# Nikhil-Kulkarni/RayTrace-miniapp

Hardware: AMD Instinct MI355X
Metric: ray_steps_per_sec (higher is better)
Workload: dtype f32+f64

## Files before the change

include/rt_hip.h:

```cpp
#ifndef RT_HIP_H
#define RT_HIP_H

#include <stddef.h>
#include <stdint.h>

#ifdef __cplusplus
extern "C" {
#endif

#define RT_N_SUB 3
#define RT_N_FAILED_MAX 32

enum {
    RT_OK            = 0,
    RT_ERR_ARG       = 1,
    RT_ERR_NO_DEVICE = 2,
    RT_ERR_HIP       = 3,
    RT_ERR_NOMEM     = 4
};

typedef struct rt_ray {
    float x, y, a, b;
} rt_ray;

// ... 70 lines not shown
                             int ngy, const double *ga, int nga, const double *gb, int ngb,
                             int64_t first, int64_t stride, int64_t count);

int rt_hip_plan_run(rt_hip_plan *plan, void *stream, double *image_dev, double *iang_dev);

int rt_hip_plan_fetch(rt_hip_plan *plan, double *image, double *I_ang,
                      unsigned int *failure_code, rt_ray *failed_rays, int max_failed,
                      int *n_failed, rt_stats *stats);

int rt_hip_plan_kernel_ms(rt_hip_plan *plan, float *ms);

int rt_hip_plan_kernel_times(rt_hip_plan *plan, float *march_ms, float *freq_ms);

int rt_hip_plan_last_fused(rt_hip_plan *plan);

int rt_hip_plan_set_timing_ring(rt_hip_plan *plan, int n_runs);
int rt_hip_plan_ring_times(rt_hip_plan *plan, float *march_ms, float *freq_ms, int max_runs, int *n_runs);

double *rt_hip_plan_image_ptr(rt_hip_plan *plan);
double *rt_hip_plan_iang_ptr(rt_hip_plan *plan);

int rt_hip_plan_enable_probe(rt_hip_plan *plan, int on);
int rt_hip_plan_fetch_probe(rt_hip_plan *plan, float *gvl, float *evl, int32_t *ivl,
                            rt_ray *ray2, uint32_t *flags, uint32_t *steps);

int rt_hip_plan_set_exact_emission(rt_hip_plan *plan, int on);

int rt_hip_plan_set_step_factor(rt_hip_plan *plan, double c);

int rt_hip_plan_enable_path(rt_hip_plan *plan, int on);
// ... 18 lines not shown
```

raytrace-miniapp_amd/backend.py:

```python
from __future__ import annotations

import ctypes as C
import subprocess
import time
from pathlib import Path

import numpy as np

from . import cabi
from .problem import Problem

CSRC = Path(__file__).resolve().parent / "csrc"
LIB_PATH = CSRC / "librt_hip.so"


class RayTraceError(RuntimeError):
    """Raised where the reference calls RAY_ERROR (utilities/RayUtilityMacros.h:88-91)."""


def build_library(force: bool = False) -> Path:
    if force and LIB_PATH.exists():
        LIB_PATH.unlink()
    subprocess.run(["make", "-s", "-C", str(CSRC)], check=True)
    return LIB_PATH
# ... 157 lines not shown
        return torch.as_tensor(v, device=torch.device("cuda", self.device))

    def kernel_ms(self) -> float:
        ms = C.c_float(0)
        self.hl.check(self.hl.lib.rt_hip_plan_kernel_ms(self._h, C.byref(ms)), "rt_hip_plan_kernel_ms")
        return float(ms.value)

    def kernel_times(self) -> tuple:
        a, f = C.c_float(0), C.c_float(0)
        self.hl.check(self.hl.lib.rt_hip_plan_kernel_times(self._h, C.byref(a), C.byref(f)),
                      "rt_hip_plan_kernel_times")
        return float(a.value), float(f.value)

    def last_fused(self) -> bool:
        return bool(self.hl.lib.rt_hip_plan_last_fused(self._h))

    def set_timing_ring(self, n_runs: int) -> "Plan":
        self.hl.check(self.hl.lib.rt_hip_plan_set_timing_ring(self._h, int(n_runs)), "rt_hip_plan_set_timing_ring")
        self._ring = int(n_runs)
        return self

    def ring_times(self) -> list:
        n = getattr(self, "_ring", 0)
        if n < 1:
            return []
        a = np.zeros(n, np.float32)
        f = np.zeros(n, np.float32)
        got = C.c_int(0)
        self.hl.check(self.hl.lib.rt_hip_plan_ring_times(self._h, cabi._fp(a), cabi._fp(f), n, C.byref(got)),
                      "rt_hip_plan_ring_times")
# ... 163 lines not shown
```

raytrace-miniapp_amd/cabi.py:

```python
from __future__ import annotations

import ctypes as C

import numpy as np

RT_N_SUB = 3
RT_N_FAILED_MAX = 32

RT_OK, RT_ERR_ARG, RT_ERR_NO_DEVICE, RT_ERR_HIP, RT_ERR_NOMEM = range(5)

c_double_p = C.POINTER(C.c_double)
c_float_p = C.POINTER(C.c_float)


class RtRay(C.Structure):
    _fields_ = [("x", C.c_float), ("y", C.c_float), ("a", C.c_float), ("b", C.c_float)]


RAY_DTYPE = np.dtype([("x", "<f4"), ("y", "<f4"), ("a", "<f4"), ("b", "<f4")])


class RtBeam(C.Structure):
    _fields_ = [
        ("nx", C.c_int32), ("ny", C.c_int32), ("na", C.c_int32), ("nb", C.c_int32),
# ... 129 lines not shown
    lib.rt_hip_plan_set_ray_grid.argtypes = [vp, c_double_p, C.c_int, c_double_p, C.c_int,
                                             c_double_p, C.c_int, c_double_p, C.c_int,
                                             C.c_int64, C.c_int64, C.c_int64]
    lib.rt_hip_plan_set_ray_grid.restype = C.c_int
    lib.rt_hip_plan_run.argtypes = [vp, vp, vp, vp]
    lib.rt_hip_plan_run.restype = C.c_int
    lib.rt_hip_plan_fetch.argtypes = [vp, c_double_p, c_double_p, P(C.c_uint), P(RtRay), C.c_int,
                                      P(C.c_int), P(RtStats)]
    lib.rt_hip_plan_fetch.restype = C.c_int
    lib.rt_hip_plan_kernel_ms.argtypes = [vp, P(C.c_float)]
    lib.rt_hip_plan_kernel_ms.restype = C.c_int
    lib.rt_hip_plan_kernel_times.argtypes = [vp, P(C.c_float), P(C.c_float)]
    lib.rt_hip_plan_kernel_times.restype = C.c_int
    lib.rt_hip_plan_last_fused.argtypes = [vp]
    lib.rt_hip_plan_last_fused.restype = C.c_int
    lib.rt_hip_plan_set_timing_ring.argtypes = [vp, C.c_int]
    lib.rt_hip_plan_set_timing_ring.restype = C.c_int
    lib.rt_hip_plan_ring_times.argtypes = [vp, c_float_p, c_float_p, C.c_int, P(C.c_int)]
    lib.rt_hip_plan_ring_times.restype = C.c_int
    lib.rt_hip_plan_image_ptr.argtypes = [vp]
    lib.rt_hip_plan_image_ptr.restype = vp
    lib.rt_hip_plan_iang_ptr.argtypes = [vp]
    lib.rt_hip_plan_iang_ptr.restype = vp
    lib.rt_hip_plan_enable_probe.argtypes = [vp, C.c_int]
    lib.rt_hip_plan_enable_probe.restype = C.c_int
    lib.rt_hip_plan_fetch_probe.argtypes = [vp, c_float_p, c_float_p, P(C.c_int32), P(RtRay),
                                            P(C.c_uint32), P(C.c_uint32)]
    lib.rt_hip_plan_fetch_probe.restype = C.c_int
    lib.rt_hip_plan_set_exact_emission.argtypes = [vp, C.c_int]
    lib.rt_hip_plan_set_exact_emission.restype = C.c_int
# ... 10 lines not shown
    lib.rt_hip_plan_spectra_ptr.argtypes = [vp]
    lib.rt_hip_plan_spectra_ptr.restype = vp
    lib.rt_hip_calc_rays.argtypes = [C.c_int, C.c_int, C.c_double, P(RtGain), P(RtSeed), C.c_int, C.c_int, c_double_p,
                                     C.c_size_t, c_double_p, c_double_p, P(C.c_int32), P(RtStats)]
    lib.rt_hip_calc_rays.restype = C.c_int
    lib.rt_hip_plan_set_debug.argtypes = [vp, C.c_uint]
    lib.rt_hip_plan_set_debug.restype = C.c_int
    lib.rt_hip_plan_destroy.argtypes = [vp]
    lib.rt_hip_plan_destroy.restype = None


HIP_API_SYMBOLS = [
    "rt_hip_device_count", "rt_hip_last_error", "rt_hip_selftest", "rt_hip_image_loop", "rt_hip_multi_image_loop",
    "rt_hip_multi_last_mode", "rt_hip_ray_list_grid_dims", "rt_hip_host_libm_mode", "rt_hip_pool_trim", "rt_hip_plan_create",
    "rt_hip_plan_set_rays", "rt_hip_plan_set_ray_grid", "rt_hip_plan_run", "rt_hip_plan_fetch",
    "rt_hip_plan_kernel_ms", "rt_hip_plan_kernel_times", "rt_hip_plan_last_fused", "rt_hip_plan_set_timing_ring", "rt_hip_plan_ring_times", "rt_hip_plan_image_ptr", "rt_hip_plan_iang_ptr", "rt_hip_plan_enable_probe",
    "rt_hip_plan_fetch_probe", "rt_hip_plan_set_exact_emission", "rt_hip_plan_set_step_factor", "rt_hip_plan_enable_path",
    "rt_hip_plan_fetch_path", "rt_hip_plan_enable_spectra", "rt_hip_plan_fetch_spectra", "rt_hip_plan_spectra_ptr",
    "rt_hip_calc_rays", "rt_hip_plan_set_debug", "rt_hip_plan_destroy",
]
```

raytrace-miniapp_amd/csrc/rt_fused.hip:

```cpp
#pragma once
#include "rt_freq.hip"

namespace rt {

struct FusedLay {
    unsigned off_exp, off_iang, off_ctl, off_rem, off_nodes, off_buf;
    unsigned node_cap;
    unsigned n_free, per_wave;
    unsigned split, k_part;
    unsigned n_consumers, consumers_first;
};
struct FusedKArg {
    DevParams P;
    FreqKArg F;
    unsigned *tile_next;
    FusedLay lay;
};

constexpr int fused_wave_doubles(int maxq) { return 4 * XP_ROW + maxq * WAVE; }
template <bool BOUNDED, int SF, int MAXQ, bool EMIS = true>
__global__ void __launch_bounds__(1024) rt_fused_kernel(const FusedKArg A)
{
    extern __shared__ __align__(16) unsigned char lds_raw[];
#ifdef RT_WAVETIMES
    if (threadIdx.x == 0)
        atomicMin(&g_wt[2], __builtin_amdgcn_s_memrealtime());
#endif
    const FreqHot &H   = A.F.hot;
    const int n_ang    = H.n_ang;
    double *exp2_tab   = reinterpret_cast<double *>(lds_raw + A.lay.off_exp);
    double *lds_iang   = reinterpret_cast<double *>(lds_raw + A.lay.off_iang);
    unsigned *ctl      = reinterpret_cast<unsigned *>(lds_raw + A.lay.off_ctl);
    double *buf_free   = reinterpret_cast<double *>(lds_raw + A.lay.off_buf);
    const unsigned n_waves  = blockDim.x >> 6;
    const unsigned n_march  = n_waves - A.lay.n_consumers;
// ... 6 lines not shown
        lds_iang[c] = 0.0;
    for (unsigned c = threadIdx.x; c < n_waves * 32u; c += blockDim.x)
        reinterpret_cast<unsigned *>(lds_raw + A.lay.off_rem)[c] = 0u;
    if (threadIdx.x == 0) {
        ctl[0] = TILE_NONE;
        ctl[1] = n_march;
        ctl[2] = 0u;
        ctl[3] = 0u;
    }
    const TileList list{ &ctl[0], A.tile_next, reinterpret_cast<unsigned *>(lds_raw + A.lay.off_nodes), &ctl[3], A.lay.node_cap,
                         reinterpret_cast<unsigned *>(lds_raw + A.lay.off_rem) + wave_id * 32u,
                         &ctl[1], n_march, A.lay.split, A.lay.k_part };

    march_load_tables<true>(A.P, lds_raw);
    if (!consumer)
        march_wave<true, BOUNDED, true, EMIS ? 1 : 0>(A.P, lds_raw, list);

    const int lane = lane_id();
#ifdef RT_WAVETIMES
    const unsigned long long fu_left = __builtin_amdgcn_s_memrealtime();
    unsigned long long fu_first = 0, fu_tiles = 0;
#endif
    unsigned slot  = 0;
    if (lane == 0) {
        if (!consumer)
            __hip_atomic_fetch_add(&ctl[1], 0xffffffffu, __ATOMIC_RELAXED, __HIP_MEMORY_SCOPE_WORKGROUP);
        slot = __hip_atomic_fetch_add(&ctl[2], 1u, __ATOMIC_RELAXED, __HIP_MEMORY_SCOPE_WORKGROUP);
    }
    slot = (unsigned) __builtin_amdgcn_readfirstlane((int) slot);
    auto marching = [&]() { return __hip_atomic_load(&ctl[1], __ATOMIC_RELAXED, __HIP_MEMORY_SCOPE_WORKGROUP); };
    double *mine;
// ... 78 lines not shown
```

raytrace-miniapp_amd/csrc/rt_launch.hip:

```cpp
#include "rt_path.hip"
#include "rt_freq.hip"
#include "rt_fused.hip"
#include "rt_spec.hip"

#include "rt_runtime.h"

#include <atomic>
#include <cstdlib>
#include <cstring>
#include <map>
#include <mutex>

using namespace rtr;

namespace {

int allow_lds(const void *kernel, int device, size_t bytes, size_t limit)
{
    static std::mutex mu;
    static std::map<std::pair<int, const void *>, size_t> allowed;
    if (bytes <= 64 * 1024)
        return RT_OK;
    std::lock_guard<std::mutex> lock(mu);
    size_t &have = allowed[{ device, kernel }];
// ... 139 lines not shown
    rt::SpecKArg a;
    memset(&a, 0, sizeof(a));
    a.hot       = f.hot;
    a.hot.image = nullptr;
    a.hot.iang  = nullptr;
    a.cold      = f.cold;
    a.out       = p->spec[p->spec_sel];
    const int rc = allow_lds(reinterpret_cast<const void *>(&rt::rt_spec_kernel<SF, EMIS>), p->device, lds, p->lds_limit);
    if (rc != RT_OK)
        return rc;
    hipLaunchKernelGGL((rt::rt_spec_kernel<SF, EMIS>), dim3(grid), dim3((unsigned) wg_waves * 64), lds, stream, a);
    HIP_TRY(hipGetLastError());
    return RT_OK;
}

int launch_spec_any(rt_hip_plan *p, hipStream_t stream)
{
    const int S = p->P.L * RT_N_SUB;
    if (p->P.use_emis)
        return (S == 6) ? launch_spec<6, true>(p, stream) : launch_spec<0, true>(p, stream);
    return (S == 6) ? launch_spec<6, false>(p, stream) : launch_spec<0, false>(p, stream);
}

}

namespace rt {
extern "C" __global__ void __launch_bounds__(256) rt_zero_kernel(unsigned long long *a, unsigned long long na, unsigned long long *b,
                                                                unsigned long long nb, unsigned long long *c, unsigned long long nc)
{
    const unsigned long long step = (unsigned long long) gridDim.x * blockDim.x;
// ... 116 lines not shown
                            p->n_iang * sizeof(double) <= 32 * 1024 && env_unsigned("RT_HIP_FUSED", 1, 1, 2) == 1;
    unsigned bthr = lds_tab ? 1024u : 256u;
    if (lds_tab && !fused_cand) {
        const unsigned long long per_cu_rays = p->cu_count ? p->n_rays / (unsigned long long) p->cu_count : 0;
        bthr = per_cu_rays >= 4ull * 1024 ? 1024u : (per_cu_rays >= 2560ull ? 768u : 512u);
    }
    bthr = env_unsigned("RT_HIP_MARCH_THREADS", bthr, 64, lds_tab ? 1024 : 256) / 64 * 64;
    const size_t mlds   = lds_tab ? (size_t) p->P.blob_bytes : 0;
    int per_cu          = 0;
    const bool force_ieee = getenv("RT_HIP_MARCH_IEEE") != nullptr;
    const bool bounded = p->tables_bounded && p->P.c_h3 >= 1e-8f && !force_ieee;
    using march_fn = void (*)(const rt::DevParams);
    int mode = (p->P.use_emis && p->P.method == 1 && !p->path_on) ? 1 : 0;
    if (!p->P.use_emis && p->P.method == 2 && !p->path_on)
        mode = (int) env_unsigned("RT_HIP_MARCH_MODE", 3, 0, 4);
    const march_fn kernel =
        lds_tab ? (bounded ? (mode == 1 ? rt::rt_march_kernel<true, true, 1> : mode == 2 ? rt::rt_march_kernel<true, true, 2> : mode == 3 ? rt::rt_march_kernel<true, true, 3> : mode == 4 ? rt::rt_march_kernel<true, true, 4> : rt::rt_march_kernel<true, true, 0>)
                           : (mode == 1 ? rt::rt_march_kernel<true, false, 1> : rt::rt_march_kernel<true, false, 0>))
                : (bounded ? rt::rt_march_kernel<false, true, 0> : rt::rt_march_kernel<false, false, 0>);
    if (lds_tab) {
        const int rc = allow_lds(reinterpret_cast<const void *>(kernel), p->device, mlds, p->lds_limit);
        if (rc != RT_OK)
            return rc;
        per_cu = 1;
        if (2 * mlds + 1024 <= p->lds_limit && bthr <= 512)
            HIP_TRY(hipOccupancyMaxActiveBlocksPerMultiprocessor(&per_cu, kernel, (int) bthr, mlds));
    } else {
        HIP_TRY(hipOccupancyMaxActiveBlocksPerMultiprocessor(&per_cu, kernel, (int) bthr, mlds));
    }
    if (per_cu < 1)
        per_cu = 1;
    unsigned long long want = ((unsigned long long) p->n_rays + bthr - 1) / bthr;
    unsigned long long cap  = (unsigned long long) p->cu_count * (unsigned) per_cu;
    const unsigned grid     = (unsigned) (want < cap ? want : cap);
// ... 102 lines not shown
            p->P.chunk     = p->P.chunk < 64 ? 64 : p->P.chunk;
            if (emis)
                late_zone(p, (unsigned) ((p->n_rays + bthr - 1) / bthr < (unsigned long long) p->cu_count ? (p->n_rays + bthr - 1) / bthr : p->cu_count),
                          nw - lay.n_consumers, lay.consumers_first ? lay.n_consumers : 0u);
            p->P.tile_begin = 0;
            p->P.tile_end   = p->P.n_tiles;
            p->P.freq_id    = 0;
            rt::FusedKArg fa;
            fa.P         = p->P;
            fa.F         = freq_args(p, true, nslot, (unsigned long long) grid * nw);
            fa.tile_next = p->tile_next;
            fa.lay       = lay;
            const int S  = p->P.L * RT_N_SUB;
            using fused_fn = void (*)(const rt::FusedKArg);
            const fused_fn fk =
                !emis     ? (S == 6 ? (bounded ? rt::rt_fused_kernel<true, 6, 3, false> : rt::rt_fused_kernel<false, 6, 3, false>)
                                    : (bounded ? rt::rt_fused_kernel<true, 0, 3, false> : rt::rt_fused_kernel<false, 0, 3, false>))
                : maxq == 2 ? (S == 6 ? (bounded ? rt::rt_fused_kernel<true, 6, 2> : rt::rt_fused_kernel<false, 6, 2>)
                                    : (bounded ? rt::rt_fused_kernel<true, 0, 2> : rt::rt_fused_kernel<false, 0, 2>))
                          : (S == 6 ? (bounded ? rt::rt_fused_kernel<true, 6, 3> : rt::rt_fused_kernel<false, 6, 3>)
                                    : (bounded ? rt::rt_fused_kernel<true, 0, 3> : rt::rt_fused_kernel<false, 0, 3>));
            {
                const int rc = allow_lds(reinterpret_cast<const void *>(fk), p->device, flds, p->lds_limit);
                if (rc != RT_OK)
                    return rc;
            }
            unsigned long long fwant = ((unsigned long long) p->n_rays + bthr - 1) / bthr;
            const unsigned fgrid     = (unsigned) (fwant < (unsigned long long) p->cu_count ? fwant : (unsigned long long) p->cu_count);
            hipLaunchKernelGGL(fk, dim3(fgrid), dim3(bthr), flds, stream, fa);
            HIP_TRY(hipGetLastError());
            p->host_rays = nullptr;
            HIP_TRY(hipEventRecord(p->evm, stream));
            HIP_TRY(hipEventRecord(p->ev1, stream));
            p->last_fused = true;
            return RT_OK;
        }
// ... 92 lines not shown
    HIP_TRY(hipMemcpyFromSymbol(n_waves, HIP_SYMBOL(rt::g_ft_n), sizeof(unsigned)));
    const unsigned zero = 0;
    HIP_TRY(hipMemcpyToSymbol(HIP_SYMBOL(rt::g_ft_n), &zero, sizeof(zero)));
    return RT_OK;
}
#endif

#ifdef RT_INSTRUMENT
int rt_hip_debug_ray_iters(unsigned short *out, unsigned long long n)
{
    HIP_TRY(hipDeviceSynchronize());
    HIP_TRY(hipMemcpyFromSymbol(out, HIP_SYMBOL(rt::g_ray_iters), (size_t) n * sizeof(unsigned short)));
    return RT_OK;
}
#endif
#if defined(RT_INSTRUMENT) || defined(RT_TIMEBLOCKS)
int rt_hip_debug_counters(unsigned long long *out8)
{
    HIP_TRY(hipDeviceSynchronize());
    HIP_TRY(hipMemcpyFromSymbol(out8, HIP_SYMBOL(rt::g_inst), 8 * sizeof(unsigned long long)));
    unsigned long long z[8] = { 0 };
    HIP_TRY(hipMemcpyToSymbol(HIP_SYMBOL(rt::g_inst), z, sizeof(z)));
    return RT_OK;
}
#endif

}
```

raytrace-miniapp_amd/csrc/rt_march.hip:

```cpp
#pragma once
#include "rt_math.h"

#include <cfloat>

namespace rt {

enum : int { ST_IDLE = 0, ST_CELL = 1, ST_XSETUP = 2, ST_STEP = 3, ST_DONE = 4 };

typedef double f64x2 __attribute__((ext_vector_type(2)));
typedef float f32x4 __attribute__((ext_vector_type(4)));
typedef unsigned u32x4 __attribute__((ext_vector_type(4)));

__device__ __forceinline__ unsigned div_magic(unsigned x, unsigned mul, unsigned sh)
{
    return mul ? __umulhi(x, mul) >> sh : x;
}
__device__ __forceinline__ void grid_index(const DevRays &R, unsigned ridx, unsigned &i, unsigned &j, unsigned &k,
                                           unsigned &m)
{
    const unsigned ijkm = (unsigned) (R.first + (long long) ridx * R.stride);
    const unsigned q1   = div_magic(ijkm, R.div_mul[0], R.div_sh[0]);
    m                   = ijkm - q1 * (unsigned) R.ngb;
    const unsigned q2   = div_magic(q1, R.div_mul[1], R.div_sh[1]);
    k                   = q1 - q2 * (unsigned) R.nga;
// ... 20 lines not shown
        if (want_tan) {
            ta = R.tan_a[k];
            tb = R.tan_b[m];
        }
    }
}

__device__ __attribute__((noinline)) float tan_wide(float x)
{
    if (!(fabsf(x) <= FLT_MAX))
        return x - x;
    return (float) tan((double) x);
}
__device__ __attribute__((noinline)) float atan_wide(float x)
{
    if (x != x)
        return x + x;
    if (!(fabsf(x) <= FLT_MAX))
        return copysignf(1.5707963705062866f, x);
    return (float) atan((double) x);
}

__device__ __attribute__((noinline)) float ktanf_flt32(float x, float y, int iy)
{
    const float T[13] = { 3.3333334327e-01f, 1.3333334029e-01f, 5.3968254477e-02f, 2.1869488060e-02f, 8.8632395491e-03f,
                          3.5920790397e-03f, 1.4562094584e-03f, 5.8804126456e-04f, 2.4646313977e-04f, 7.8179444245e-05f,
                          7.1407252108e-05f, -1.8558637748e-05f, 2.5907305826e-05f };
    const float pio4 = 7.8539812565e-01f, pio4lo = 3.7748947079e-08f;
    float z, r, v, w, s;
    const int hx = (int) __float_as_uint(x), ix = hx & 0x7fffffff;
    if (ix < 0x39000000) {
        if ((int) x == 0) {
            if ((ix | (iy + 1)) == 0)
                return 1.0f / fabsf(x);
            else if (iy == 1)
// ... 315 lines not shown
            for (int u = 0; u < 8; u++) {
                const unsigned i = i0 + (unsigned) u * step;
                v[u]             = src[i < n16 ? i : i0];
            }
#pragma unroll
            for (int u = 0; u < 8; u++) {
                const unsigned i = i0 + (unsigned) u * step;
                if (i < n16)
                    dst[i] = v[u];
            }
        }
        __syncthreads();
    }
}

template <bool LDS_TAB, bool BOUNDED, bool FUSED, int MODE = 0>
__device__ __forceinline__ void march_wave(const DevParams &P, unsigned char *lds_raw, const TileList done)
{
    const int lane        = lane_id();
    const int L           = P.L;
    const int S           = L * RT_N_SUB;
    const unsigned n_rays = P.ray_end;
    const bool backward   = MODE == 1 ? true : ((MODE == 2 || MODE == 3) ? false : P.method == 1);
    const bool use_emis   = MODE == 1 ? true : ((MODE == 2 || MODE == 4) ? false : P.use_emis != 0);
    const bool path_on    = MODE == 0 ? P.path_on != 0 : false;
    const unsigned CH     = P.chunk;
#ifndef RT_REFILL
#define RT_REFILL 8
#endif
    const int REFILL      = RT_REFILL;

// ... 1 lines not shown
    const BlobGain *hdr = reinterpret_cast<const BlobGain *>(tab);
    const unsigned lds_base = LDS_TAB ? (unsigned) (size_t) (__attribute__((address_space(3))) unsigned char *) lds_raw : 0u;

    static_assert(RT_N_SUB == 3, "sub-segment ends are tabulated for three sub-segments");
    float zs0 = (P.dz0 * (0.0f + 1.0f) / RT_N_SUB), zs1 = (P.dz0 * (1.0f + 1.0f) / RT_N_SUB),
          zs2 = (P.dz0 * (2.0f + 1.0f) / RT_N_SUB);
    asm volatile("" : "+v"(zs0), "+v"(zs1), "+v"(zs2));

    unsigned chunk_next = 0, chunk_end = 0;
    unsigned fetched_end = 0, slot_busy = 0, cur_slot = 0;
    unsigned cslot       = 0;
    bool more           = true;
    const unsigned n_launch_rays = n_rays - P.ray_begin;
    const unsigned n_chunks      = (n_launch_rays + CH - 1) / CH;
    unsigned shard = blockIdx.x & 7u, shards_seen_empty = 0;
    const unsigned n_main = n_chunks - (P.late_chunks < n_chunks ? P.late_chunks : 0u);
    const bool late_wave  = (unsigned) __builtin_amdgcn_readfirstlane((int) (threadIdx.x >> 6)) - P.late_first < P.late_waves;
    unsigned zone = 0;

    int st        = ST_IDLE;
    unsigned ridx = 0;
    int seg = 0, iz = 0, ii = 0;
    float z = 0.0f, z_stop = 0.0f;
    float px = 0, py = 0, pz = 0, sx = 0, sy = 0, sz = 1;
    float gacc = 0, eacc = 0;
    int cell_last = 0, sub = 0;
    unsigned char *recp = P.rec;
    unsigned lane12     = 0;
    BlobGain G    = hdr[1];
    unsigned steps = 0;
    bool escaped = false, mirror = false;
// ... 502 lines not shown
                        float g = gxn;
                        asm volatile("" : "+v"(g));
                        qx = g / n;
                    }
                    if (fabsf(gyn) < 1e-29f && gyn != 0.0f) {
                        float g = gyn;
                        asm volatile("" : "+v"(g));
                        qy = g / n;
                    }
                }
#endif
                float fx = qx - sx * t;
                float fy = qy - sy * t;
                float fz = -sz * t;
                float h;
                if (BOUNDED) {
                    const float h1 = fdiv_nr(P.c_h1, fabsf(t));
                    const float h2 = fdiv_nr(1.0001f * (lim2 - fabsf(rz)), fabsf(sz));
                    const float h3 = fdiv_nr(P.c_h3 * (fabsf(sx) + 5e-4f), (fabsf(fx) + 1e-8f));
                    const float h4 = fdiv_nr(P.c_h3 * (fabsf(sy) + 5e-4f), (fabsf(fy) + 1e-8f));
                    h = fmin_nan_drop(fmin_nan_drop(h1, dzcap), fmin_nan_drop(h2, fmin_nan_drop(h3, h4)));
                } else {
                    h        = RT_FDIV(P.c_h1, fabsf(t));
                    h        = h < dzcap ? h : dzcap;
                    float h2 = RT_FDIV(1.0001f * (lim2 - fabsf(rz)), fabsf(sz));
                    float h3 = RT_FDIV(P.c_h3 * (fabsf(sx) + 5e-4f), (fabsf(fx) + 1e-8f));
                    float h4 = RT_FDIV(P.c_h3 * (fabsf(sy) + 5e-4f), (fabsf(fy) + 1e-8f));
                    h        = h < h2 ? h : h2;
                    h        = h < h3 ? h : h3;
                    h        = h < h4 ? h : h4;
                }
                float ht = h * t;
                const float R3 = 1.0f / 3.0f, R6 = 1.0f / 6.0f, R12 = 1.0f / 12.0f;
                float c1 = 0.5f * h * h * (1.0f - div_by_recip<true>(ht, 3.0f, R3) + div_by_recip<true>(ht * ht, 12.0f, R12));
                rx += sx * h + c1 * fx;
                ry += sy * h + c1 * fy;
                rz += sz * h + c1 * fz;
                float c2 = h * (1.0f - 0.5f * ht + div_by_recip<true>(ht * ht, 6.0f, R6));
                sx += c2 * fx;
                sy += c2 * fy;
                sz += c2 * fz;
                renormalise(sx, sy, sz);
                hsum += h;
                RT_TICK(0);
                run = (fabsf(rx) < lim0) & (fabsf(ry) < lim1) & (fabsf(rz) < lim2) & (fabsf(n - n0) < 0.05f);
            }
            if (!run) {
                path += hsum;
                px += rx;
                py += ry;
                pz += rz;
                zc += fabsf(rz);
                const float ya = mirror ? fabsf(py) : py;
                if ((px > ix1.y) & (px < ix1.z) & (ya > iy1.y) & (ya < iy1.z) & ((double) zc < 0.999 * (double) dzrem)) {
                    st = ST_XSETUP;
                } else {
                    z += fabsf(pz);
                    gacc += g0 * path;
                    eacc += E0 * path;
                    cell_last = c00;
// ... 41 lines not shown
            atomicAdd(&g_inst[7], tb_iters);
        }
#endif
#ifdef RT_INSTRUMENT
        for (int i = 0; i < 3; i++) {
            unsigned tw = wave_sum_u32(inst.w[i]), ta = wave_sum_u32(inst.a[i]);
            if (lane == 0) {
                atomicAdd(&g_inst[2 * i], (unsigned long long) tw);
                atomicAdd(&g_inst[2 * i + 1], (unsigned long long) ta);
            }
        }
#endif
    }
}

template <bool LDS_TAB, bool BOUNDED, int MODE = 0>
__global__ void __launch_bounds__(LDS_TAB ? 1024 : 256) rt_march_kernel(const DevParams P)
{
    extern __shared__ __align__(16) unsigned char lds_raw[];
    march_load_tables<LDS_TAB>(P, lds_raw);
    march_wave<LDS_TAB, BOUNDED, false, MODE>(P, lds_raw, TileList{ nullptr, nullptr, nullptr, nullptr, 0u, nullptr, nullptr, 0u, 0u, 0u });
}

}
```

raytrace-miniapp_amd/csrc/rt_math.h:

```cpp
#pragma once

#include "rt_device.h"

namespace rt {

#ifdef RT_INSTRUMENT
__device__ unsigned long long g_inst[8];
struct Inst {
    unsigned w[3] = { 0, 0, 0 }, a[3] = { 0, 0, 0 };
    __device__ __forceinline__ void tick(int i)
    {
        a[i]++;
        unsigned long long m = __ballot(1);
        if ((int) (threadIdx.x & 63) == __ffsll((long long) m) - 1)
            w[i]++;
    }
};
#define RT_TICK(i) inst.tick(i)
#else
#define RT_TICK(i)
#endif
#if defined(RT_TIMEBLOCKS) || defined(RT_WAVEBLOCKS)
#ifndef RT_INSTRUMENT
__device__ unsigned long long g_inst[8];
// ... 206 lines not shown
```

raytrace-miniapp_amd/csrc/rt_plan.hip:

```cpp
#include "rt_runtime.h"

#include <algorithm>
#include <cfloat>
#include <cmath>
#include <cstdio>
#include <cstdlib>
#include <cstring>
#include <memory>
#include <mutex>
#include <string>
#include <thread>

using namespace rtr;

namespace {

struct ArenaBuilder {
    unsigned char *base = nullptr;
    size_t cap = 0, used = 0;
    bool pinned = false, overflow = false;
    std::unique_ptr<unsigned char[]> own;
    ArenaBuilder() = default;
    ArenaBuilder(const ArenaBuilder &) = delete;
    ArenaBuilder &operator=(const ArenaBuilder &) = delete;
// ... 286 lines not shown
            if (i == 4 && seed->dim[4] != K) {
                delete p;
                return fail_arg("rt_hip_plan_create: seed.dim[4] != beam.nv");
            }
            off_sx[i] = ab.put(seed->x[i], sizeof(double) * (size_t) seed->dim[i]);
            if (i == 4) {
                off_sf[i] = ab.reserve(sizeof(double) * (size_t) Kp);
                memcpy(ab.base + off_sf[i], seed->f[i], sizeof(double) * (size_t) seed->dim[i]);
            } else {
                off_sf[i] = ab.put(seed->f[i], sizeof(double) * (size_t) seed->dim[i]);
            }
        }
    }
    const size_t off_gain = ab.reserve(sizeof(rt::DevGain) * (size_t) N);
    std::vector<unsigned char> blob(align_up(sizeof(rt::BlobGain) * (size_t) N, 16));
    bool tiny_spacing = false, bad_index = false, all_bounded = true;
    for (int i = 1; i < N; i++) {
        const rt_gain &g  = gain[i];
        const size_t npix = (size_t) g.Nx * (size_t) g.Ny;
        rt::BlobGain h;
        memset(&h, 0, sizeof(h));
        h.lo_x     = (float) g.x[0];
        h.hi_x     = (float) g.x[g.Nx - 1];
        h.lo_y     = (float) g.y[0];
        h.hi_y     = (float) g.y[g.Ny - 1];
        h.mirror_y = 0;
        if (h.lo_y >= 0) {
            h.lo_y     = -h.hi_y;
            h.mirror_y = 1;
        }
        h.Nx     = g.Nx;
// ... 45 lines not shown
            for (int k = 1; k < g.Ny; k++)
                w_min = std::min(w_min, g.y[k] - g.y[k - 1]);
            for (int iy = 0; iy < g.Ny; iy++) {
                const double *row = g.n + (size_t) iy * (size_t) g.Nx;
                for (int ix = 0; ix < g.Nx; ix++) {
                    n_lo = std::min(n_lo, row[ix]);
                    n_hi = std::max(n_hi, row[ix]);
                    if (ix > 0)
                        dn = std::max(dn, fabs(row[ix] - row[ix - 1]));
                    if (iy > 0)
                        dn = std::max(dn, fabs(row[ix] - row[ix - g.Nx]));
                }
            }
            if (!(n_lo - dn >= 0.25 && n_hi + dn <= 4.0 && dn / w_min <= 1e12 && w_min >= 1e-12))
                all_bounded = false;
        }
    }
    if (!(beam->dz >= 1e-12 && beam->dz <= 1e6))
        all_bounded = false;
    p->tables_bounded = all_bounded;
    if (tiny_spacing) {
        delete p;
        return fail_arg("rt_hip_plan_create: gain grid not strictly increasing, or spacing below 1e-30");
    }
    if (bad_index) {
        delete p;
        return fail_arg("rt_hip_plan_create: non-finite index of refraction");
    }
    const size_t off_blob = ab.put(blob.data(), blob.size());
    lap("pack");

#define PLAN_TRY(expr)                                   \
    do {                                                 \
        hipError_t e_ = (expr);                          \
        if (e_ != hipSuccess) {                          \
// ... 603 lines not shown
    return RT_OK;
}

int rt_hip_plan_kernel_times(rt_hip_plan *p, float *march_ms, float *freq_ms)
{
    if (!p || !p->ran || !march_ms || !freq_ms)
        return fail_arg("rt_hip_plan_kernel_times: plan has not run");
    HIP_TRY(hipSetDevice(p->device));
    HIP_TRY(hipEventSynchronize(p->ev1));
    HIP_TRY(hipEventElapsedTime(march_ms, p->ev0, p->evm));
    HIP_TRY(hipEventElapsedTime(freq_ms, p->evm, p->ev1));
    return RT_OK;
}

int rt_hip_plan_last_fused(rt_hip_plan *p) { return p && p->ran && p->last_fused ? 1 : 0; }

double *rt_hip_plan_image_ptr(rt_hip_plan *p) { return p ? p->image_own : nullptr; }
double *rt_hip_plan_iang_ptr(rt_hip_plan *p) { return p ? p->iang_own : nullptr; }

int rt_hip_plan_fetch_probe(rt_hip_plan *p, float *gvl, float *evl, int32_t *ivl, rt_ray *ray2,
                            uint32_t *flags, uint32_t *steps)
{
    if (!p || !p->ran || !p->probe_on || !p->probe)
        return fail_arg("rt_hip_plan_fetch_probe: probe was not enabled for the last run");
    HIP_TRY(hipSetDevice(p->device));
    HIP_TRY(hipStreamSynchronize(p->last_stream));
    const size_t n = (size_t) p->n_rays, S = (size_t) p->P.L * RT_N_SUB;
    {
        std::vector<unsigned char> h(rt::rec_bytes(n, p->P.rec_stride));
        if (n)
// ... 201 lines not shown
```

raytrace-miniapp_amd/csrc/rt_runtime.h:

```cpp
#pragma once

#include "rt_device.h"
#include "rt_spec.h"

#include <chrono>
#include <string>
#include <vector>

struct rt_hip_plan {
    int device         = 0;
    int cu_count       = 0;
    rt::DevParams P    = {};
    unsigned char *arena = nullptr;
    size_t arena_bytes = 0;
    void *staging        = nullptr;
    hipStream_t upload_q = nullptr;
    unsigned char *out_staging = nullptr;
    bool out_staged            = false;
    rt_ray *rays_dev   = nullptr;
    double *grid_dev   = nullptr;
    float *tan_dev     = nullptr;
    double *seedtab_dev = nullptr;
    std::vector<double> beam_x, beam_y, beam_a, beam_b;
    unsigned char *rec = nullptr;
// ... 22 lines not shown
    hipStream_t last_stream = nullptr;
    hipStream_t queued_stream = nullptr;
    bool queued = false;
    double *last_image = nullptr, *last_iang = nullptr;
    bool ran = false;
    std::vector<hipEvent_t> ring;
    unsigned long long runs = 0;
    bool repeated = false;
    unsigned char *bad_dev = nullptr;
    size_t bad_rays        = 0;
    std::chrono::steady_clock::time_point t_created;
    std::vector<const float *> gv_dev;
    const double *dv2_dev = nullptr;
    bool gv_has_nan       = false;
    bool tables_bounded   = false;
    unsigned *tile_next   = nullptr;
    size_t tile_next_n    = 0;
    bool last_fused       = false;
    size_t lds_limit      = 0;
};

namespace rtr {

std::string &last_error();
int fail_hip(hipError_t e, const char *what, const char *file, int line);
int fail_arg(const char *msg);

#define HIP_TRY(expr)                                                \
    do {                                                             \
        hipError_t e_ = (expr);                                      \
// ... 47 lines not shown
```

Measured before the change: 29.30 billion.

## Prune step-size divisions wave-uniformly and drop proven refractive-index test in bounded march

Adds templated march and fused kernel variants that skip the h1 and h2/h4 step-size divisions when a wave-wide ballot shows they cannot bind against the dz cap. The variants also drop the per-step |n-n0| termination test when plan creation proves it cannot trigger. Separately, atan_wide is replaced with a float polynomial (fdlibm-style) instead of a double atan call. The goal is fewer divides and fewer double-precision ops per ray step, at the cost of more kernel instantiations and reliance on the conservative proof margins.

```diff
diff --git a/include/rt_hip.h b/include/rt_hip.h
--- a/include/rt_hip.h
+++ b/include/rt_hip.h
@@ -108,6 +108,8 @@
 
 int rt_hip_plan_last_fused(rt_hip_plan *plan);
 
+int rt_hip_plan_last_march_instance(rt_hip_plan *plan);
+
 int rt_hip_plan_set_timing_ring(rt_hip_plan *plan, int n_runs);
 int rt_hip_plan_ring_times(rt_hip_plan *plan, float *march_ms, float *freq_ms, int max_runs, int *n_runs);
 
diff --git a/raytrace-miniapp_amd/backend.py b/raytrace-miniapp_amd/backend.py
--- a/raytrace-miniapp_amd/backend.py
+++ b/raytrace-miniapp_amd/backend.py
@@ -195,6 +195,9 @@
 
     def last_fused(self) -> bool:
         return bool(self.hl.lib.rt_hip_plan_last_fused(self._h))
+
+    def last_march_instance(self) -> int:
+        return int(self.hl.lib.rt_hip_plan_last_march_instance(self._h))
 
     def set_timing_ring(self, n_runs: int) -> "Plan":
         self.hl.check(self.hl.lib.rt_hip_plan_set_timing_ring(self._h, int(n_runs)), "rt_hip_plan_set_timing_ring")
diff --git a/raytrace-miniapp_amd/cabi.py b/raytrace-miniapp_amd/cabi.py
--- a/raytrace-miniapp_amd/cabi.py
+++ b/raytrace-miniapp_amd/cabi.py
@@ -167,6 +167,9 @@
     lib.rt_hip_plan_kernel_times.restype = C.c_int
     lib.rt_hip_plan_last_fused.argtypes = [vp]
     lib.rt_hip_plan_last_fused.restype = C.c_int
+    if hasattr(lib, "rt_hip_plan_last_march_instance"):
+        lib.rt_hip_plan_last_march_instance.argtypes = [vp]
+        lib.rt_hip_plan_last_march_instance.restype = C.c_int
     lib.rt_hip_plan_set_timing_ring.argtypes = [vp, C.c_int]
     lib.rt_hip_plan_set_timing_ring.restype = C.c_int
     lib.rt_hip_plan_ring_times.argtypes = [vp, c_float_p, c_float_p, C.c_int, P(C.c_int)]
@@ -207,7 +210,7 @@
     "rt_hip_device_count", "rt_hip_last_error", "rt_hip_selftest", "rt_hip_image_loop", "rt_hip_multi_image_loop",
     "rt_hip_multi_last_mode", "rt_hip_ray_list_grid_dims", "rt_hip_host_libm_mode", "rt_hip_pool_trim", "rt_hip_plan_create",
     "rt_hip_plan_set_rays", "rt_hip_plan_set_ray_grid", "rt_hip_plan_run", "rt_hip_plan_fetch",
-    "rt_hip_plan_kernel_ms", "rt_hip_plan_kernel_times", "rt_hip_plan_last_fused", "rt_hip_plan_set_timing_ring", "rt_hip_plan_ring_times", "rt_hip_plan_image_ptr", "rt_hip_plan_iang_ptr", "rt_hip_plan_enable_probe",
+    "rt_hip_plan_kernel_ms", "rt_hip_plan_kernel_times", "rt_hip_plan_last_fused", "rt_hip_plan_last_march_instance", "rt_hip_plan_set_timing_ring", "rt_hip_plan_ring_times", "rt_hip_plan_image_ptr", "rt_hip_plan_iang_ptr", "rt_hip_plan_enable_probe",
     "rt_hip_plan_fetch_probe", "rt_hip_plan_set_exact_emission", "rt_hip_plan_set_step_factor", "rt_hip_plan_enable_path",
     "rt_hip_plan_fetch_path", "rt_hip_plan_enable_spectra", "rt_hip_plan_fetch_spectra", "rt_hip_plan_spectra_ptr",
     "rt_hip_calc_rays", "rt_hip_plan_set_debug", "rt_hip_plan_destroy",
diff --git a/raytrace-miniapp_amd/csrc/rt_fused.hip b/raytrace-miniapp_amd/csrc/rt_fused.hip
--- a/raytrace-miniapp_amd/csrc/rt_fused.hip
+++ b/raytrace-miniapp_amd/csrc/rt_fused.hip
@@ -18,7 +18,7 @@
 };
 
 constexpr int fused_wave_doubles(int maxq) { return 4 * XP_ROW + maxq * WAVE; }
-template <bool BOUNDED, int SF, int MAXQ, bool EMIS = true>
+template <bool BOUNDED, int SF, int MAXQ, bool EMIS = true, int OPT = 0>
 __global__ void __launch_bounds__(1024) rt_fused_kernel(const FusedKArg A)
 {
     extern __shared__ __align__(16) unsigned char lds_raw[];
@@ -55,7 +55,7 @@
 
     march_load_tables<true>(A.P, lds_raw);
     if (!consumer)
-        march_wave<true, BOUNDED, true, EMIS ? 1 : 0>(A.P, lds_raw, list);
+        march_wave<true, BOUNDED, true, EMIS ? 1 : 0, OPT>(A.P, lds_raw, list);
 
     const int lane = lane_id();
 #ifdef RT_WAVETIMES
diff --git a/raytrace-miniapp_amd/csrc/rt_launch.hip b/raytrace-miniapp_amd/csrc/rt_launch.hip
--- a/raytrace-miniapp_amd/csrc/rt_launch.hip
+++ b/raytrace-miniapp_amd/csrc/rt_launch.hip
@@ -177,6 +177,15 @@
     return RT_OK;
 }
 
+template <bool LDS_TAB, int MODE> void (*march_bounded(int opt))(const rt::DevParams)
+{
+    return opt == 7 ? rt::rt_march_kernel<LDS_TAB, true, MODE, 7> : opt == 3 ? rt::rt_march_kernel<LDS_TAB, true, MODE, 3> : rt::rt_march_kernel<LDS_TAB, true, MODE, 0>;
+}
+template <int SF, int MAXQ, bool EMIS> void (*fused_bounded(int opt))(const rt::FusedKArg)
+{
+    return opt == 7 ? rt::rt_fused_kernel<true, SF, MAXQ, EMIS, 7> : opt == 3 ? rt::rt_fused_kernel<true, SF, MAXQ, EMIS, 3> : rt::rt_fused_kernel<true, SF, MAXQ, EMIS, 0>;
+}
+
 int launch_spec_any(rt_hip_plan *p, hipStream_t stream)
 {
     const int S = p->P.L * RT_N_SUB;
@@ -323,10 +332,15 @@
     int mode = (p->P.use_emis && p->P.method == 1 && !p->path_on) ? 1 : 0;
     if (!p->P.use_emis && p->P.method == 2 && !p->path_on)
         mode = (int) env_unsigned("RT_HIP_MARCH_MODE", 3, 0, 4);
+    const unsigned long long launch_rays = p->n_rays / n_launch;
+    const bool prune_h24 = p->march_prune == 2 || (p->cu_count && launch_rays / (unsigned long long) p->cu_count >= 8192ull);
+    const int opt = (bounded && p->march_prune && p->ntest_proven)
+                        ? (rt::MARCH_OPT_PRUNE | rt::MARCH_OPT_NO_NTEST | (prune_h24 ? rt::MARCH_OPT_PRUNE_H24 : 0)) : 0;
+    p->last_march_inst = (bounded ? 1 : 0) | (opt << 1);
     const march_fn kernel =
-        lds_tab ? (bounded ? (mode == 1 ? rt::rt_march_kernel<true, true, 1> : mode == 2 ? rt::rt_march_kernel<true, true, 2> : mode == 3 ? rt::rt_march_kernel<true, true, 3> : mode == 4 ? rt::rt_march_kernel<true, true, 4> : rt::rt_march_kernel<true, true, 0>)
+        lds_tab ? (bounded ? (mode == 1 ? march_bounded<true, 1>(opt) : mode == 2 ? march_bounded<true, 2>(opt) : mode == 3 ? march_bounded<true, 3>(opt) : mode == 4 ? march_bounded<true, 4>(opt) : march_bounded<true, 0>(opt))
                            : (mode == 1 ? rt::rt_march_kernel<true, false, 1> : rt::rt_march_kernel<true, false, 0>))
-                : (bounded ? rt::rt_march_kernel<false, true, 0> : rt::rt_march_kernel<false, false, 0>);
+                : (bounded ? march_bounded<false, 0>(opt) : rt::rt_march_kernel<false, false, 0>);
     if (lds_tab) {
         const int rc = allow_lds(reinterpret_cast<const void *>(kernel), p->device, mlds, p->lds_limit);
         if (rc != RT_OK)
@@ -459,12 +473,12 @@
             const int S  = p->P.L * RT_N_SUB;
             using fused_fn = void (*)(const rt::FusedKArg);
             const fused_fn fk =
-                !emis     ? (S == 6 ? (bounded ? rt::rt_fused_kernel<true, 6, 3, false> : rt::rt_fused_kernel<false, 6, 3, false>)
-                                    : (bounded ? rt::rt_fused_kernel<true, 0, 3, false> : rt::rt_fused_kernel<false, 0, 3, false>))
-                : maxq == 2 ? (S == 6 ? (bounded ? rt::rt_fused_kernel<true, 6, 2> : rt::rt_fused_kernel<false, 6, 2>)
-                                    : (bounded ? rt::rt_fused_kernel<true, 0, 2> : rt::rt_fused_kernel<false, 0, 2>))
-                          : (S == 6 ? (bounded ? rt::rt_fused_kernel<true, 6, 3> : rt::rt_fused_kernel<false, 6, 3>)
-                                    : (bounded ? rt::rt_fused_kernel<true, 0, 3> : rt::rt_fused_kernel<false, 0, 3>));
+                !emis     ? (S == 6 ? (bounded ? fused_bounded<6, 3, false>(opt) : rt::rt_fused_kernel<false, 6, 3, false>)
+                                    : (bounded ? fused_bounded<0, 3, false>(opt) : rt::rt_fused_kernel<false, 0, 3, false>))
+                : maxq == 2 ? (S == 6 ? (bounded ? fused_bounded<6, 2, true>(opt) : rt::rt_fused_kernel<false, 6, 2>)
+                                    : (bounded ? fused_bounded<0, 2, true>(opt) : rt::rt_fused_kernel<false, 0, 2>))
+                          : (S == 6 ? (bounded ? fused_bounded<6, 3, true>(opt) : rt::rt_fused_kernel<false, 6, 3>)
+                                    : (bounded ? fused_bounded<0, 3, true>(opt) : rt::rt_fused_kernel<false, 0, 3>));
             {
                 const int rc = allow_lds(reinterpret_cast<const void *>(fk), p->device, flds, p->lds_limit);
                 if (rc != RT_OK)
@@ -587,6 +601,16 @@
     return RT_OK;
 }
 #endif
+#ifdef RT_INSTRUMENT
+int rt_hip_debug_prune_counters(unsigned long long *out4)
+{
+    HIP_TRY(hipDeviceSynchronize());
+    HIP_TRY(hipMemcpyFromSymbol(out4, HIP_SYMBOL(rt::g_prune), 4 * sizeof(unsigned long long)));
+    unsigned long long z[4] = { 0 };
+    HIP_TRY(hipMemcpyToSymbol(HIP_SYMBOL(rt::g_prune), z, sizeof(z)));
+    return RT_OK;
+}
+#endif
 #if defined(RT_INSTRUMENT) || defined(RT_TIMEBLOCKS)
 int rt_hip_debug_counters(unsigned long long *out8)
 {
diff --git a/raytrace-miniapp_amd/csrc/rt_march.hip b/raytrace-miniapp_amd/csrc/rt_march.hip
--- a/raytrace-miniapp_amd/csrc/rt_march.hip
+++ b/raytrace-miniapp_amd/csrc/rt_march.hip
@@ -58,11 +58,45 @@
 }
 __device__ __attribute__((noinline)) float atan_wide(float x)
 {
-    if (x != x)
-        return x + x;
-    if (!(fabsf(x) <= FLT_MAX))
-        return copysignf(1.5707963705062866f, x);
-    return (float) atan((double) x);
+    const float A0 = 3.3333334327e-01f, A1 = -2.0000000298e-01f, A2 = 1.4285714924e-01f, A3 = -1.1111110449e-01f,
+                A4 = 9.0908870101e-02f, A5 = -7.6918758452e-02f, A6 = 6.6610731184e-02f, A7 = -5.8335702866e-02f,
+                A8 = 4.9768779427e-02f, A9 = -3.6531571299e-02f, A10 = 1.6285819933e-02f;
+    const unsigned hx = __float_as_uint(x), ix = hx & 0x7fffffffu;
+    const bool neg = (hx >> 31) != 0u;
+    if (ix >= 0x4c000000u) {
+        if (ix > 0x7f800000u)
+            return x + x;
+        const float r = 1.5707962513e+00f + 7.5497894159e-08f;
+        return neg ? -r : r;
+    }
+    float hi, lo;
+    x = fabsf(x);
+    if (ix < 0x3f980000u) {
+        if (ix < 0x3f300000u) {
+            hi = 4.6364760399e-01f;
+            lo = 5.0121582440e-09f;
+            x  = (2.0f * x - 1.0f) / (2.0f + x);
+        } else {
+            hi = 7.8539812565e-01f;
+            lo = 3.7748947079e-08f;
+            x  = (x - 1.0f) / (x + 1.0f);
+        }
+    } else {
+        if (ix < 0x401c0000u) {
+            hi = 9.8279368877e-01f;
+            lo = 3.4473217170e-08f;
+            x  = (x - 1.5f) / (1.0f + 1.5f * x);
+        } else {
+            hi = 1.5707962513e+00f;
+            lo = 7.5497894159e-08f;
+            x  = -1.0f / x;
+        }
+    }
+    const float z = x * x, w = z * z;
+    const float s1 = z * (A0 + w * (A2 + w * (A4 + w * (A6 + w * (A8 + w * A10)))));
+    const float s2 = w * (A1 + w * (A3 + w * (A5 + w * (A7 + w * A9))));
+    const float r  = hi - ((x * (s1 + s2) - lo) - x);
+    return neg ? -r : r;
 }
 
 __device__ __attribute__((noinline)) float ktanf_flt32(float x, float y, int iy)
@@ -408,7 +442,8 @@
     }
 }
 
-template <bool LDS_TAB, bool BOUNDED, bool FUSED, int MODE = 0>
+enum : int { MARCH_OPT_PRUNE = 1, MARCH_OPT_NO_NTEST = 2, MARCH_OPT_PRUNE_H24 = 4 };
+template <bool LDS_TAB, bool BOUNDED, bool FUSED, int MODE = 0, int OPT = 0>
 __device__ __forceinline__ void march_wave(const DevParams &P, unsigned char *lds_raw, const TileList done)
 {
     const int lane        = lane_id();
@@ -440,7 +475,11 @@
     const unsigned n_launch_rays = n_rays - P.ray_begin;
     const unsigned n_chunks      = (n_launch_rays + CH - 1) / CH;
     unsigned shard = blockIdx.x & 7u, shards_seen_empty = 0;
+#ifdef RT_MARCH_ONE_COUNTER
+    const unsigned n_main = n_chunks;
+#else
     const unsigned n_main = n_chunks - (P.late_chunks < n_chunks ? P.late_chunks : 0u);
+#endif
     const bool late_wave  = (unsigned) __builtin_amdgcn_readfirstlane((int) (threadIdx.x >> 6)) - P.late_first < P.late_waves;
     unsigned zone = 0;
 
@@ -973,7 +1012,32 @@
                 float fy = qy - sy * t;
                 float fz = -sz * t;
                 float h;
-                if (BOUNDED) {
+                if (BOUNDED && (OPT & MARCH_OPT_PRUNE)) {
+                    const float kd = 1.00002f * dzcap;
+                    const float at = fabsf(t), az = fabsf(sz);
+                    const float n2 = 1.0001f * (lim2 - fabsf(rz));
+                    const float n4 = P.c_h3 * (fabsf(sy) + 5e-4f), d4 = fabsf(fy) + 1e-8f;
+                    h = fmin_nan_drop(fdiv_nr(P.c_h3 * (fabsf(sx) + 5e-4f), (fabsf(fx) + 1e-8f)), dzcap);
+#ifdef RT_INSTRUMENT
+                    const bool cnt_lane = lane == (int) __ffsll((long long) __ballot(1)) - 1;
+                    if (cnt_lane)
+                        atomicAdd(&g_prune[3], 1ull);
+#endif
+                    if (__ballot(!(P.c_h1 > kd * at)) != 0ull) {
+                        h = fmin_nan_drop(fdiv_nr(P.c_h1, at), h);
+#ifdef RT_INSTRUMENT
+                        if (cnt_lane)
+                            atomicAdd(&g_prune[0], 1ull);
+#endif
+                    }
+                    if (!(OPT & MARCH_OPT_PRUNE_H24) || __ballot(!(n2 > kd * az) | !(n4 > kd * d4)) != 0ull) {
+                        h = fmin_nan_drop(fmin_nan_drop(fdiv_nr(n2, az), fdiv_nr(n4, d4)), h);
+#ifdef RT_INSTRUMENT
+                        if (cnt_lane)
+                            atomicAdd(&g_prune[1], 1ull);
+#endif
+                    }
+                } else if (BOUNDED) {
                     const float h1 = fdiv_nr(P.c_h1, fabsf(t));
                     const float h2 = fdiv_nr(1.0001f * (lim2 - fabsf(rz)), fabsf(sz));
                     const float h3 = fdiv_nr(P.c_h3 * (fabsf(sx) + 5e-4f), (fabsf(fx) + 1e-8f));
@@ -1002,7 +1066,9 @@
                 renormalise(sx, sy, sz);
                 hsum += h;
                 RT_TICK(0);
-                run = (fabsf(rx) < lim0) & (fabsf(ry) < lim1) & (fabsf(rz) < lim2) & (fabsf(n - n0) < 0.05f);
+                run = (fabsf(rx) < lim0) & (fabsf(ry) < lim1) & (fabsf(rz) < lim2);
+                if (!(BOUNDED && (OPT & MARCH_OPT_NO_NTEST)))
+                    run = run & (fabsf(n - n0) < 0.05f);
             }
             if (!run) {
                 path += hsum;
@@ -1074,12 +1140,12 @@
     }
 }
 
-template <bool LDS_TAB, bool BOUNDED, int MODE = 0>
+template <bool LDS_TAB, bool BOUNDED, int MODE = 0, int OPT = 0>
 __global__ void __launch_bounds__(LDS_TAB ? 1024 : 256) rt_march_kernel(const DevParams P)
 {
     extern __shared__ __align__(16) unsigned char lds_raw[];
     march_load_tables<LDS_TAB>(P, lds_raw);
-    march_wave<LDS_TAB, BOUNDED, false, MODE>(P, lds_raw, TileList{ nullptr, nullptr, nullptr, nullptr, 0u, nullptr, nullptr, 0u, 0u, 0u });
-}
-
-}
+    march_wave<LDS_TAB, BOUNDED, false, MODE, OPT>(P, lds_raw, TileList{ nullptr, nullptr, nullptr, nullptr, 0u, nullptr, nullptr, 0u, 0u, 0u });
+}
+
+}
diff --git a/raytrace-miniapp_amd/csrc/rt_math.h b/raytrace-miniapp_amd/csrc/rt_math.h
--- a/raytrace-miniapp_amd/csrc/rt_math.h
+++ b/raytrace-miniapp_amd/csrc/rt_math.h
@@ -6,6 +6,7 @@
 
 #ifdef RT_INSTRUMENT
 __device__ unsigned long long g_inst[8];
+__device__ unsigned long long g_prune[4];
 struct Inst {
     unsigned w[3] = { 0, 0, 0 }, a[3] = { 0, 0, 0 };
     __device__ __forceinline__ void tick(int i)
diff --git a/raytrace-miniapp_amd/csrc/rt_plan.hip b/raytrace-miniapp_amd/csrc/rt_plan.hip
--- a/raytrace-miniapp_amd/csrc/rt_plan.hip
+++ b/raytrace-miniapp_amd/csrc/rt_plan.hip
@@ -324,7 +324,7 @@
     }
     const size_t off_gain = ab.reserve(sizeof(rt::DevGain) * (size_t) N);
     std::vector<unsigned char> blob(align_up(sizeof(rt::BlobGain) * (size_t) N, 16));
-    bool tiny_spacing = false, bad_index = false, all_bounded = true;
+    bool tiny_spacing = false, bad_index = false, all_bounded = true, ntest_proven = true;
     for (int i = 1; i < N; i++) {
         const rt_gain &g  = gain[i];
         const size_t npix = (size_t) g.Nx * (size_t) g.Ny;
@@ -400,11 +400,16 @@
             }
             if (!(n_lo - dn >= 0.25 && n_hi + dn <= 4.0 && dn / w_min <= 1e12 && w_min >= 1e-12))
                 all_bounded = false;
+            const double fy = g.y[0] >= 0.0 ? std::max(1.2, 1.0 + 2.0 * g.y[0] / (g.y[1] - g.y[0])) : 1.2;
+            if (!(8.0 * 0.1 * (1.2 + fy) * dn <= 0.05 - 1e-5))
+                ntest_proven = false;
         }
     }
     if (!(beam->dz >= 1e-12 && beam->dz <= 1e6))
         all_bounded = false;
     p->tables_bounded = all_bounded;
+    p->ntest_proven   = all_bounded && ntest_proven;
+    p->march_prune    = (int) env_unsigned("RT_HIP_MARCH_PRUNE", 1, 0, 2);
     if (tiny_spacing) {
         delete p;
         return fail_arg("rt_hip_plan_create: gain grid not strictly increasing, or spacing below 1e-30");
@@ -1038,6 +1043,7 @@
 }
 
 int rt_hip_plan_last_fused(rt_hip_plan *p) { return p && p->ran && p->last_fused ? 1 : 0; }
+int rt_hip_plan_last_march_instance(rt_hip_plan *p) { return p && p->ran ? p->last_march_inst : 0; }
 
 double *rt_hip_plan_image_ptr(rt_hip_plan *p) { return p ? p->image_own : nullptr; }
 double *rt_hip_plan_iang_ptr(rt_hip_plan *p) { return p ? p->iang_own : nullptr; }
diff --git a/raytrace-miniapp_amd/csrc/rt_runtime.h b/raytrace-miniapp_amd/csrc/rt_runtime.h
--- a/raytrace-miniapp_amd/csrc/rt_runtime.h
+++ b/raytrace-miniapp_amd/csrc/rt_runtime.h
@@ -60,6 +60,9 @@
     const double *dv2_dev = nullptr;
     bool gv_has_nan       = false;
     bool tables_bounded   = false;
+    bool ntest_proven     = false;
+    int march_prune       = 1;
+    int last_march_inst   = 0;
     unsigned *tile_next   = nullptr;
     size_t tile_next_n    = 0;
     bool last_fused       = false;
```

Measured after the change: 29.85 billion (median of 6 runs). 1.9% higher.
